# ConsenSys/wittgenstein

Hardware: NVIDIA H100
Metric: simulated-ms/sec, GSFSignature 65,536 nodes (higher is better)
Workload: dtype u64 bitmaps / int32

## Files before the change

wittgenstein_b200/csrc/wtg_cuda.cu:

```cuda
#include <cuda_runtime.h>
#include <unistd.h>

#include <cstdio>
#include <cstdlib>
#include <stdexcept>
#include <string>
#include <vector>

#include "wtg_engine.hpp"

namespace wtg {

#define CUDA_OK(x)                                                                                       \
  do {                                                                                                   \
    cudaError_t e_ = (x);                                                                                \
    if (e_ != cudaSuccess) throw std::runtime_error(std::string("CUDA: ") + cudaGetErrorString(e_) + " at " #x); \
  } while (0)

constexpr int SCAN_THREADS = 256;
constexpr int SCAN_ITEMS = 4;
constexpr int SCAN_TILE = SCAN_THREADS * SCAN_ITEMS;

__global__ void k_begin(Dev d, int mode, bool condAhead) {
  if (threadIdx.x >= 32) return;
  if (d.ffwd && mode == 1) {
    CoopWarp c;
    tickBeginFfwd(d, c);
  } else if (d.farCap > 0 && !d.ffwd) {
    CoopWarp c;
    tickBeginFar(d, c, mode, condAhead);
  } else if (threadIdx.x == 0) {
    tickBegin(d, mode, condAhead);
  }
}
__global__ void k_end(Dev d, int mode, bool condAhead) {
  if (threadIdx.x == 0) tickEnd(d, mode, condAhead);
}
__global__ void k_cond_begin(Dev d) {
  if (threadIdx.x == 0) condBegin(d);
}

__device__ __forceinline__ void listAppend(const Dev& d, bool active, int n, int* cnt, int* list, u64* words = nullptr, u64 word = 0) {
  CoopWarp c;
  unsigned m = c.ballot(active);
  if (!m) return;
  int stripe = ((blockIdx.x * blockDim.x + threadIdx.x) >> 5) & (ARENA_STRIPES - 1);
  int base = 0;
  if (c.lane() == 0) base = atomicAdd(&cnt[stripe], c.count(m));
  base = c.bcast(base, 0);
  if (active) {
    size_t at = (size_t)stripe * d.listStripeCap + base + c.rank(m);
    list[at] = n;
    if (words) words[at] = word;
  }
}
__global__ void __launch_bounds__(256) k_cond_mark(Dev d) {
  if (d.ctl->error) return;
  const int blk = blockIdx.x;
  int n = d.n0 + blk * blockDim.x + threadIdx.x;
  bool due = false;
  if (n < d.n0 + d.nLoc) due = d.proto == PROTO_HANDEL ? hCondMark(d, n) : gsfCondMark(d, n);
  listAppend(d, due, n, d.ctl->dueCnt, d.dueList);
}
template <int PHASE>
__global__ void __launch_bounds__(256) k_cond_nodes(Dev d) {
  extern __shared__ uint32_t keepAll[];
  __shared__ HScratch scratch[8];
  if (d.ctl->error) return;
  const int blk = blockIdx.x, nBlk = gridDim.x;
  const int stripe = blk & (ARENA_STRIPES - 1);
  const int cnt = d.ctl->dueCnt[stripe];
  const int warp = threadIdx.x >> 5;
  const int sub = (blk >> 6) * 8 + warp;
  const int nsub = (nBlk >> 6) * 8;
  const int* list = d.dueList + (size_t)stripe * d.listStripeCap;
  CoopWarp c;
  for (int t = sub; t < cnt; t += nsub) {
    int n = list[t];
    if (PHASE == 0) {
      if (d.proto == PROTO_HANDEL)
        hCondScanQueue(d, c, n);
      else
        gsfCondScanQueue(d, c, n);
    } else {
      if (d.proto == PROTO_HANDEL)
        hCondSelect(d, c, n, &scratch[warp]);
      else
        gsfCondSelect(d, c, n, keepAll + (size_t)warp * (size_t)(d.qcap / 32));
    }
  }
}
__global__ void __launch_bounds__(256) k_cond_score(Dev d) {
  if (d.ctl->error) return;
  const int blk = blockIdx.x, nBlk = gridDim.x;
  const int per = d.workCap / ARENA_STRIPES;
  const int stripe = blk & (ARENA_STRIPES - 1);
  int cnt = d.ctl->workCnt[stripe];
  if (cnt > per) cnt = per;
  const int warpsPerBlock = blockDim.x >> 5;
  const int sub = (blk >> 6) * warpsPerBlock + (threadIdx.x >> 5);
  const int nsub = (nBlk >> 6) * warpsPerBlock;
  CoopWarp c;
  const uint32_t* wl = d.workList + (size_t)stripe * per;
  for (int t = sub; t < cnt; t += nsub) {
    uint32_t it = wl[t];
    if (d.proto == PROTO_HANDEL)
      hScoreItem(d, c, it);
    else
      gsfScoreItem(d, c, it);
  }
}
__global__ void k_hpick_check(Dev d) {
  if (d.ctl->error) return;
  const int blk = blockIdx.x, nBlk = gridDim.x;
  for (int n = d.n0 + blk * blockDim.x + threadIdx.x; n < d.n0 + d.nLoc; n += nBlk * blockDim.x)
    if (d.hCandK[n] > 0 && (d.forcePickSerial || hCondPick(d, n, (u64)d.hDrawBase[n], false) > d.condDraws[n])) d.ctl->hReject = 1;
}
__global__ void k_hpick_apply(Dev d) {
  if (d.ctl->error) return;
  const int blk = blockIdx.x, nBlk = gridDim.x;
  if (!d.ctl->hReject) {
    for (int n = d.n0 + blk * blockDim.x + threadIdx.x; n < d.n0 + d.nLoc; n += nBlk * blockDim.x) hCondPick(d, n, (u64)d.hDrawBase[n], true);
  } else if (blk == 0 && threadIdx.x == 0) {
    u64 idx = 0;
    for (int n = d.n0; n < d.n0 + d.nLoc; ++n) idx += (u64)hCondPick(d, n, idx, true);
  }
}
__global__ void k_hpick_publish(Dev d) {
  const int blk = blockIdx.x, nBlk = gridDim.x;
  if (!d.ctl->error)
    for (int n = d.n0 + blk * blockDim.x + threadIdx.x; n < d.n0 + d.nLoc; n += nBlk * blockDim.x) hPickPublish(d, n);
  if (blk == 0 && threadIdx.x == 0) hPickPublishHeader(d);
}
__global__ void k_hpick_xcheck(Dev d) {
  if (d.ctl->error) return;
  const int blk = blockIdx.x, nBlk = gridDim.x;
  if (blk == 0 && threadIdx.x == 0) hPickHeaders(d);
  const int upTo = hPicksBelow(d, d.rank + 1);
  for (int t = blk * blockDim.x + threadIdx.x; t < upTo; t += nBlk * blockDim.x)
    if (hPickRejects(d, t)) d.ctl->hReject = 1;
}
__global__ void k_hpick_xapply(Dev d) {
  if (d.ctl->error) return;
  const int blk = blockIdx.x, nBlk = gridDim.x;
  if (!d.ctl->hReject) {
    const u64 below = (u64)hPicksBelow(d, d.rank);
    for (int n = d.n0 + blk * blockDim.x + threadIdx.x; n < d.n0 + d.nLoc; n += nBlk * blockDim.x) hCondPick(d, n, below + (u64)d.hDrawBase[n], true);
  } else if (blk == 0 && threadIdx.x == 0) {
    hPickSerial(d);
  }
// ... 383 lines not shown
  }
}
__global__ void __launch_bounds__(256) k_ms_scatter(Dev d) {
  extern __shared__ int msHist[];
  if (d.ctl->error) return;
  const int blk = blockIdx.x, nBlk = gridDim.x;
  const int G = d.ctl->totalSlots, tick = d.ctl->tick, ring = d.ring;
  const int W = d.msWarps, CH = W * MS_SUB;
  const int nChunks = (G + CH - 1) / CH;
  const int warp = threadIdx.x >> 5, lane = threadIdx.x & 31;
  int* base = msHist + warp * ring;
  CoopWarp cw;
  for (int ch = blk; ch < nChunks; ch += nBlk) {
    msZero(msHist, ring, W);
    __syncthreads();
    const int g0 = ch * CH + warp * MS_SUB;
    int tg[MS_ROUNDS];
    msWarpHistogram(d, base, g0, G, tick, lane, tg);
    __syncthreads();
    const int* row = d.msCount + (size_t)ch * ring;
    for (int b = threadIdx.x; b < ring; b += blockDim.x) {
      int run = row[b];
      for (int w = 0; w < W; ++w) {
        int c = msHist[w * ring + b];
        msHist[w * ring + b] = run;
        run += c;
      }
    }
    __syncthreads();
#pragma unroll
    for (int r = 0; r < MS_ROUNDS; ++r) {
      int g = g0 + r * 32 + lane;
      int t = tg[r];
      int pos = cw.claim(base, t - tick, t >= 0);
      if (t >= 0) {
        if (pos < d.bcap) {
          const int4* src = reinterpret_cast<const int4*>(d.newEv + g);
          int4* dst = reinterpret_cast<int4*>(d.buckets + (size_t)(t & (ring - 1)) * (size_t)d.bcap + pos);
          int4 x = src[0], y = src[1];
          dst[0] = x;
          dst[1] = y;
          if (d.G > 1) d.bucketKey[(size_t)(t & (ring - 1)) * (size_t)d.bcap + pos] = orderKey((unsigned)d.ctl->xseq, (unsigned)g);
        }
        if (d.G > 1) d.newTarget[g] = -1;
      }
      __syncwarp();
    }
    __syncthreads();
  }
}

__global__ void k_free(Dev d) {
  if (d.ctl->error) return;
  const int blk = blockIdx.x, nBlk = gridDim.x;
  const int per = d.freeCap / ARENA_STRIPES;
  const int stripe = blk & (ARENA_STRIPES - 1);
  int cnt = d.ctl->freeCnt[stripe];
  if (cnt > per) cnt = per;
  const int sub = (blk >> 6) * blockDim.x + threadIdx.x;
  const int nsub = (nBlk >> 6) * blockDim.x;
  for (int j = sub; j < cnt; j += nsub) freeApply(d, stripe * per + j);
}

__global__ void k_gsf_init_nodes(Dev d) {
  int n = d.n0 + blockIdx.x * blockDim.x + threadIdx.x;
  if (n < d.n0 + d.nLoc) gsfInitNodeBody(d, n);
}
__global__ void k_rng_candidates(Dev d, u64 s0, u64 count, u64 chunk, int maxBound, u64* out, int* outCount, int cap) {
  u64 t = (u64)blockIdx.x * blockDim.x + threadIdx.x;
  u64 start = t * chunk;
  if (start >= count) return;
  u64 len = start + chunk <= count ? chunk : count - start;
  rngCandidateChunk(d, s0, start, len, maxBound, out, outCount, cap);
}
template <class PeerT>
__global__ void k_gsf_shuffle(Dev d, int l, u64 s0, const int* liveRank, const u64* rejOrd, int nRej) {
  int n = d.n0 + blockIdx.x * blockDim.x + threadIdx.x;
  if (n < d.n0 + d.nLoc) gsfShuffleLevel<PeerT>(d, n, l, s0, liveRank, rejOrd, nRej);
}

class CudaBackend : public Backend {
 public:
  cudaStream_t st = nullptr;
  cudaStream_t side = nullptr;
  cudaEvent_t forkEv = nullptr, joinEv = nullptr;
  int devId = 0;
  void bind() const { cudaSetDevice(devId); }
  int sms = 132;
  int smemOptin = 0;
  enum { SHAPE_PLAIN, SHAPE_FIRST, SHAPE_LAST, SHAPE_MIDDLE, NSHAPES };
  cudaGraphExec_t tickGraph[NSHAPES] = {};
  long long shapeKernels[NSHAPES] = {};
  const void* graphFor = nullptr;
  bool useGraph = true;
  long long launches = 0;
  cudaEvent_t tm0 = nullptr, tm1 = nullptr;
  enum ProfSlot { P_BEGIN, P_COND_SCAN, P_DISPATCH_COUNT, P_SCAN_PARTIAL, P_EXCHANGE, P_SCAN_FINAL, P_DISPATCH_SCATTER, P_NODE,
                  P_EMIT, P_MS_COUNT, P_MS_SCAN, P_MS_SCATTER, P_FREE, P_END, P_COND_SCORE, P_COND_SELECT, P_EMIT_PEERS,
                  P_SCAN_A_PARTIAL, P_SCAN_A_FINAL, NK };
  bool profiling = false;
  bool profSplitScans = false;
  std::vector<cudaEvent_t> evPool;
  std::vector<int> evKernel;
  size_t evUsed = 0;
  double profMs[NK] = {};
  long long profCnt[NK] = {};
  const char* profNames[NK] = {"k_begin", "k_cond_scan", "k_dispatch_count", "k_scan_partial", "k_exchange", "k_scan_final",
                               "k_dispatch_scatter", "k_node", "k_emit", "k_ms_count", "k_ms_scan", "k_ms_scatter", "k_free",
                               "k_end", "k_cond_score", "k_cond_select", "k_emit_peers", "k_scan_a_partial", "k_scan_a_final"};

  explicit CudaBackend(int requested = -1) {
    int dev = 0;
    const char* e = std::getenv("LOCAL_RANK");
    int cnt = 0;
    CUDA_OK(cudaGetDeviceCount(&cnt));
    if (cnt == 0) throw std::runtime_error("no CUDA device");
    if (e) dev = std::atoi(e) % cnt;
    const char* e2 = std::getenv("WTG_DEVICE");
    if (e2) dev = std::atoi(e2) % cnt;
    if (requested >= 0) {
      if (requested >= cnt) throw std::invalid_argument("CUDA device " + std::to_string(requested) + " does not exist");
      dev = requested;
    }
    CUDA_OK(cudaSetDevice(dev));
    devId = dev;
    cudaDeviceProp p;
    CUDA_OK(cudaGetDeviceProperties(&p, dev));
    sms = p.multiProcessorCount;
    CUDA_OK(cudaStreamCreateWithFlags(&st, cudaStreamNonBlocking));
    CUDA_OK(cudaStreamCreateWithFlags(&side, cudaStreamNonBlocking));
    CUDA_OK(cudaEventCreateWithFlags(&forkEv, cudaEventDisableTiming));
    CUDA_OK(cudaEventCreateWithFlags(&joinEv, cudaEventDisableTiming));
    CUDA_OK(cudaDeviceGetAttribute(&smemOptin, cudaDevAttrMaxSharedMemoryPerBlockOptin, dev));
    CUDA_OK(cudaFuncSetAttribute(k_ms_count, cudaFuncAttributeMaxDynamicSharedMemorySize, smemOptin));
    CUDA_OK(cudaFuncSetAttribute(k_ms_scatter, cudaFuncAttributeMaxDynamicSharedMemorySize, smemOptin));
    const char* g = std::getenv("WTG_NO_GRAPH");
    if (g && g[0] == '1') useGraph = false;
  }
  ~CudaBackend() override {
    for (void* q : ipcOpened) cudaIpcCloseMemHandle(q);
    for (cudaGraphExec_t g : tickGraph)
      if (g) cudaGraphExecDestroy(g);
    if (forkEv) cudaEventDestroy(forkEv);
    if (joinEv) cudaEventDestroy(joinEv);
    if (side) cudaStreamDestroy(side);
    if (st) cudaStreamDestroy(st);
  }
  void* alloc(size_t bytes) override {
    bind();
    void* p = nullptr;
    cudaError_t e = cudaMalloc(&p, bytes);
    if (e != cudaSuccess) throw std::runtime_error("cudaMalloc of " + std::to_string(bytes) + " bytes failed: " + cudaGetErrorString(e));
    CUDA_OK(cudaMemsetAsync(p, 0, bytes, st));
    return p;
  }
  void release(void* p) override { cudaFree(p); }
  int deviceId() const override { return devId; }
  void exportShared(void* p, unsigned char* handle) override {
    bind();
    std::memset(handle, 0, 128);
    cudaIpcMemHandle_t ih;
    CUDA_OK(cudaIpcGetMemHandle(&ih, p));
// ... 80 lines not shown
    for (int i = 0; i < shown && k < cap; ++i, ++k) {
      ms[k] = profMs[i];
      cnt[k] = profCnt[i];
      names[k] = profNames[i];
      const int a = i == P_SCAN_PARTIAL ? P_SCAN_A_PARTIAL : i == P_SCAN_FINAL ? P_SCAN_A_FINAL : -1;
      if (!profSplitScans && a >= 0) {
        ms[k] += profMs[a];
        cnt[k] += profCnt[a];
      }
    }
    return k;
  }
  void drainProfile() {
    for (size_t i = 0; i < evUsed; ++i) {
      float ms = 0;
      cudaEventElapsedTime(&ms, evPool[2 * i], evPool[2 * i + 1]);
      profMs[evKernel[i]] += ms;
      profCnt[evKernel[i]] += 1;
    }
    evUsed = 0;
  }
  void profBegin(int kid) {
    if (!profiling) return;
    if (evUsed * 2 + 2 > evPool.size()) {
      if (evUsed >= 8192) {
        CUDA_OK(cudaStreamSynchronize(st));
        drainProfile();
      } else {
        cudaEvent_t a, b;
        CUDA_OK(cudaEventCreate(&a));
        CUDA_OK(cudaEventCreate(&b));
        evPool.push_back(a);
        evPool.push_back(b);
        evKernel.push_back(0);
      }
    }
    evKernel[evUsed] = kid;
    CUDA_OK(cudaEventRecord(evPool[2 * evUsed], st));
  }
  void profEnd() {
    if (!profiling) return;
    CUDA_OK(cudaEventRecord(evPool[2 * evUsed + 1], st));
    ++evUsed;
  }

  void fork() {
    CUDA_OK(cudaEventRecord(forkEv, st));
    CUDA_OK(cudaStreamWaitEvent(side, forkEv, 0));
  }
  void join() {
    CUDA_OK(cudaEventRecord(joinEv, side));
    CUDA_OK(cudaStreamWaitEvent(st, joinEv, 0));
  }
  void enqueueCond(const Dev& d, cudaStream_t s) {
    const int wide = sms * 8;
    const size_t smem8 = d.proto == PROTO_GSF ? (size_t)8 * (size_t)(d.qcap / 32) * sizeof(uint32_t) : 0;
    profBegin(P_COND_SCAN);
    k_cond_mark<<<(d.nLoc + 255) / 256, 256, 0, s>>>(d);
    k_cond_nodes<0><<<ARENA_STRIPES * 19, 256, 0, s>>>(d);
    profEnd();
    profBegin(P_COND_SCORE);
    k_cond_score<<<ARENA_STRIPES * 19, 256, 0, s>>>(d);
    profEnd();
    profBegin(P_COND_SELECT);
    k_cond_nodes<1><<<ARENA_STRIPES * 19, 256, smem8, s>>>(d);
    profEnd();
    launches += 4;
    if (d.proto == PROTO_HANDEL) {
      Dev dd = d;
      dd.scanPartial = d.drawScanPartial;
      profBegin(P_SCAN_PARTIAL);
      k_scan_partial<<<wide, SCAN_THREADS, 0, s>>>(dd, 2);
      profEnd();
      profBegin(P_SCAN_FINAL);
      k_scan_final<<<wide, SCAN_THREADS, 0, s>>>(dd, 2);
      profEnd();
      if (d.G > 1) {
        profBegin(P_EXCHANGE);
        k_hpick_publish<<<sms, 256, 0, s>>>(d);
        k_x_sync<<<1, 32, 0, s>>>(d, 3);
        profEnd();
        profBegin(P_COND_SELECT);
        k_hpick_xcheck<<<sms, 256, 0, s>>>(d);
        k_hpick_xapply<<<sms, 256, 0, s>>>(d);
        profEnd();
        launches += 5;
      } else {
        profBegin(P_COND_SELECT);
        k_hpick_check<<<sms, 256, 0, s>>>(d);
        k_hpick_apply<<<sms, 256, 0, s>>>(d);
        profEnd();
        launches += 3;
      }
    }
  }
  void enqueueTick(const Dev& d, int mode, bool ownCond = true, bool nextCond = false) {
    const int wide = sms * 8;
    const size_t msSmem = (size_t)d.msWarps * d.ring * sizeof(int);
    const bool branches = mode == 1 && !profiling && d.G == 1 && (d.proto == PROTO_GSF || d.proto == PROTO_HANDEL);
    const bool condBranch = branches && ownCond;
    cudaStream_t sd = condBranch ? side : st;
    if (mode != 3) {
      profBegin(P_BEGIN);
      k_begin<<<1, 32, 0, st>>>(d, mode, !ownCond);
      profEnd();
    }
    if (condBranch) fork();
    if ((d.proto == PROTO_GSF || d.proto == PROTO_HANDEL) && mode != 3 && ownCond) enqueueCond(d, st);
    if (mode != 2 && mode != 3) {
      profBegin(P_DISPATCH_COUNT);
      k_dispatch_count<<<wide, 256, 0, sd>>>(d);
      profEnd();
      profBegin(P_SCAN_A_PARTIAL);
      k_scan_partial<<<wide, SCAN_THREADS, 0, sd>>>(d, 0);
      profEnd();
      profBegin(P_SCAN_A_FINAL);
      k_scan_final<<<wide, SCAN_THREADS, 0, sd>>>(d, 0);
      profEnd();
      profBegin(P_DISPATCH_SCATTER);
      k_dispatch_scatter<<<wide, 256, 0, sd>>>(d);
      profEnd();
      if (condBranch) join();
      profBegin(P_NODE);
      k_node_msgs<<<(d.nLoc + 255) / 256, 256, 0, st>>>(d);
      k_node_tasks<<<ARENA_STRIPES * 19, 256, 0, st>>>(d);
      if (d.proto == PROTO_CASPER) {
        k_casper_fixups<<<1, 32, 0, st>>>(d);
        launches += 1;
      }
      profEnd();
      launches += 6;
    }
    const bool pooled = d.proto == PROTO_GSF || d.proto == PROTO_HANDEL;
    if (nextCond) {
      fork();
      k_free<<<ARENA_STRIPES * 2, 256, 0, side>>>(d);
      k_cond_begin<<<1, 1, 0, side>>>(d);
      enqueueCond(d, side);
      launches += 2;
    }
    profBegin(P_SCAN_PARTIAL);
    k_scan_partial<<<wide, SCAN_THREADS, 0, st>>>(d, 1);
    profEnd();
    profBegin(P_SCAN_FINAL);
    k_scan_final<<<wide, SCAN_THREADS, 0, st>>>(d, 1);
    profEnd();
    if (d.G > 1) {
      profBegin(P_EXCHANGE);
      k_x1_publish<<<sms * 2, 256, 0, st>>>(d);
      k_x_sync<<<1, 32, 0, st>>>(d, 0);
      k_x1_totals<<<1, 1, 0, st>>>(d);
      k_x1_offsets<<<sms * 2, 256, 0, st>>>(d);
      profEnd();
      launches += 4;
    }
    profBegin(P_EMIT);
    if (d.shufCap > 0) {
      k_shuffle_check<<<ARENA_STRIPES * 4, 256, 0, st>>>(d);
      k_shuffle_serial<<<1, 1, 0, st>>>(d);
      launches += 2;
    }
    k_emit<<<ARENA_STRIPES * 16, 256, 0, st>>>(d);
    if (d.allCap > 0) {
      if (d.G > 1)
        k_x_all_publish<<<8, 128, 0, st>>>(d);
      else
        k_emit_all<<<d.allWarps / 4, 128, 0, st>>>(d);
      launches += 1;
    }
    profEnd();
    if (d.proto == PROTO_P2PFLOOD) {
      profBegin(P_EMIT_PEERS);
      k_emit_peers<<<sms * 8, 128, 0, st>>>(d);
      profEnd();
      launches += 1;
    }
    if (d.G > 1) {
      profBegin(P_EXCHANGE);
      k_x_sync<<<1, 32, 0, st>>>(d, 1);
      k_x2_ingest<<<sms * 4, 256, 0, st>>>(d);
      launches += 2;
      if (d.allCap > 0) {
        k_x_all_build<<<d.allWarps / 4, 128, 0, st>>>(d);
        launches += 1;
      }
      profEnd();
    }
    if (branches && !nextCond) fork();
    profBegin(P_MS_COUNT);
    k_ms_count<<<sms * 2, d.msWarps * 32, msSmem, st>>>(d);
    profEnd();
    profBegin(P_MS_SCAN);
// ... 116 lines not shown
```

wittgenstein_b200/csrc/wtg_engine.hpp:

```cpp
#pragma once
#include <chrono>
#include <cstdio>
#include <functional>
#include <thread>
#include <cstdlib>
#include <cstring>
#include <memory>
#include <string>
#include <vector>

#include "wtg_host.hpp"
#include "wtg_logic.cuh"
#include "wtg_types.h"

namespace wtg {

struct GsfParams {
  int nodeCount, threshold, pairingTime, timeoutPerLevelMs, periodDurationMs, acceleratedCallsCount, nodesDown;
};

struct SfParams {
  int nodeCount, threshold, pairingTime, signatureSize, replyTimeout, candidateCount;
};

// ... 1506 lines not shown
      int fan = 0;
      if (hs.sendTime != 0) {
        if (hs.sendTime <= time) throw std::invalid_argument("sendTime <= time");
        ds.aux |= DESC_SENDTIME;
        ds.target = hs.sendTime;
      }
      if (hs.delay < 0 || hs.delay >= (1 << 20)) throw std::invalid_argument("delaysBetweenMessage");
      if (hs.delay > 0 && hs.to.size() < 2) throw std::invalid_argument("a delay between messages needs several destinations");
      ds.aux |= (uint32_t)hs.delay << DESC_DELAY_SHIFT;
      if (hs.to.empty()) {
        if (d.allCap <= 0) throw std::logic_error("sendAll from the host needs a protocol with the sendAll path (CasperIMD)");
        ds.dkind = DK_SEND_ALL;
        ds.evKind = EV_MULTI;
        ds.nDest = (uint32_t)d.N;
        ds.target = hs.sendTime != 0 ? hs.sendTime : time + 1;
        ds.aux = 0;
        allList.push_back(i);
        fan = d.N;
      } else if (hs.to.size() == 1) {
        if (hs.to[0] < 0 || hs.to[0] >= d.N) throw std::invalid_argument("The to node is not in the network");
        ds.dkind = DK_SEND_SINGLE;
        ds.to = (uint32_t)hs.to[0];
        ds.nDest = 1;
        fan = 1;
      } else {
        ds.dkind = DK_SEND_MULTI;
        ds.to = (uint32_t)scratch.size();
        ds.nDest = (uint32_t)hs.to.size();
        for (int t : hs.to) {
          if (t < 0 || t >= d.N) throw std::invalid_argument("The to node is not in the network");
          scratch.push_back((uint32_t)t);
        }
        if ((int)hs.to.size() > MAX_ACC) scratch.insert(scratch.end(), hs.to.size(), 0u);
        fan = (int)hs.to.size();
      }
      descs[(size_t)i] = ds;
      sent[(size_t)hs.from] += fan;
      bytes[(size_t)hs.from] += (long long)fan * msgSizeOf(hs.meta);
    }
    if ((int)scratch.size() > d.destScratchCap || (int)allList.size() > d.allCap)
      throw std::runtime_error("too many destinations in one call");
    c.tick = time;
    c.condMode = 0;
    c.nEv = 0;
    c.nItems = n;
    c.totalSlots = c.totalDraws = 0;
    c.hReject = 0;
    c.shufReject = 0;
    c.allCnt = (int)allList.size();
    c.nextEvent = 0;
    const int per = d.descCap / ARENA_STRIPES;
    for (int t = 0; t < ARENA_STRIPES; ++t) {
      c.descCnt[t] = std::max(0, std::min(per, n - t * per));
      c.destCnt[t] = c.workCnt[t] = c.dueCnt[t] = c.taskCnt[t] = 0;
    }
    be->upload(d.desc, descs.data(), descs.size() * sizeof(Desc));
    std::vector<int> ones((size_t)n, 1), zerosN((size_t)d.N, 0);
    be->upload(d.evSlots, ones.data(), ones.size() * sizeof(int));
    be->upload(d.evDraws, ones.data(), ones.size() * sizeof(int));
    be->upload(d.condFired + condHalf(d, time), zerosN.data(), zerosN.size() * sizeof(int));
    if (!scratch.empty()) be->upload(d.destScratch, scratch.data(), scratch.size() * sizeof(uint32_t));
    if (!allList.empty()) be->upload(d.allList, allList.data(), allList.size() * sizeof(int));
    {
      std::vector<long long> ms((size_t)d.N), bs((size_t)d.N);
      be->download(ms.data(), d.msgSent, ms.size() * sizeof(long long));
      be->download(bs.data(), d.bytesSent, bs.size() * sizeof(long long));
      for (int i = 0; i < d.N; ++i) {
        ms[(size_t)i] += sent[(size_t)i];
        bs[(size_t)i] += bytes[(size_t)i];
      }
      be->upload(d.msgSent, ms.data(), ms.size() * sizeof(long long));
      be->upload(d.bytesSent, bs.data(), bs.size() * sizeof(long long));
    }
    writeCtl(c);
    be->tick(d, 3);
    c = readCtl();
    if (c.error) throwDeviceError(c);
  }

  int runMs(int ms) {
    requireInited();
    if (sharded() && !linked) throw std::logic_error("node-sharded network: link the shards' exchange regions before runMs");
    if (ms <= 0) throw std::invalid_argument("Should be greater than 0. ms=" + std::to_string(ms));
    long long endAt = (long long)time + ms;
    if (endAt > 0x7fffffffLL) throw std::runtime_error("Maximum time reached!");
    Ctl c = readCtl();
    if (c.error) throwDeviceError(c);
    c.until = (int)endAt;
    c.callId += 1;
    c.didSomething = 0;
    if (d.ffwd) {
      if (c.nextEvent > endAt) {
        c.time = (int)endAt;
        writeCtl(c);
        time = (int)endAt;
        return 0;
      }
      c.idle = 0;
      writeCtl(c);
      int grow = 8;
      for (long long done = 0;;) {
        int batch = (int)std::min<long long>(grow, std::max<long long>(1, ms - done));
        if (grow < 64) grow *= 2;
        runWindow(0, batch, 0);
        done += batch;
        c = readCtl();
        if (c.error) throwDeviceError(c);
        if (c.idle) break;
// ... 234 lines not shown
```

wittgenstein_b200/csrc/wtg_logic.cuh:

```cuda
#pragma once
#include "wtg_types.h"

template <class T, class U>
static inline T wtg_host_fetch_add(T* p, U v) {
  T o = *p;
  *p = (T)(o + (T)v);
  return o;
}
template <class T>
static inline T wtg_host_fetch_max(T* p, T v) {
  T o = *p;
  if (v > o) *p = v;
  return o;
}
template <class T>
static inline T wtg_host_fetch_min(T* p, T v) {
  T o = *p;
  if (v < o) *p = v;
  return o;
}
template <class T>
static inline T wtg_host_cas(T* p, T a, T b) {
  T o = *p;
  if (o == a) *p = b;
// ... 352 lines not shown
}
#if defined(__CUDACC__)
__device__ __forceinline__ void poolCounts(CoopWarp& c, const u64* sig, const u64* rowV, const u64* rowI, int nw, int& cWI, int& cWIV,
                                           int& inter, int& interI) {
  const ulonglong2* s2 = reinterpret_cast<const ulonglong2*>(sig);
  const ulonglong2* v2 = reinterpret_cast<const ulonglong2*>(rowV);
  const ulonglong2* i2 = reinterpret_cast<const ulonglong2*>(rowI);
  const int n2 = nw >> 1;
  for (int w0 = c.lane(); w0 < n2; w0 += 128) {
    ulonglong2 sv[4], vv[4], iv[4];
#pragma unroll
    for (int u = 0; u < 4; ++u) {
      int w = w0 + 32 * u;
      if (w < n2) {
        sv[u] = s2[w];
        vv[u] = v2[w];
        iv[u] = i2[w];
      } else {
        sv[u] = make_ulonglong2(0, 0);
        vv[u] = sv[u];
        iv[u] = sv[u];
      }
    }
#pragma unroll
    for (int u = 0; u < 4; ++u) {
      cWI += __popcll(iv[u].x | sv[u].x) + __popcll(iv[u].y | sv[u].y);
      cWIV += __popcll(iv[u].x | sv[u].x | vv[u].x) + __popcll(iv[u].y | sv[u].y | vv[u].y);
      inter |= ((sv[u].x & vv[u].x) | (sv[u].y & vv[u].y)) != 0;
      interI |= ((sv[u].x & iv[u].x) | (sv[u].y & iv[u].y)) != 0;
    }
  }
}
#endif

template <class C>
WTG_HD int gsfScorePool(const Dev& d, C& c, int n, uint32_t from, uint32_t meta, u64 pl) {
  int l = (int)metaLevel(meta);
  int size = 1 << (l - 1);
  int cV = d.cntVer[n * d.L + l];
  if (cV >= size) return 0;
  Blk b = levelBlock((int)from, l);
  const u64* rowV = d.verified + (size_t)n * d.W64 + b.w0;
  const u64* rowI = d.indivVer + (size_t)n * d.W64 + b.w0;
  const u64* sig = d.pool[l] + (size_t)(uint32_t)pl * (size_t)b.nw;
  int cWI = 0, cWIV = 0, inter = 0, interI = 0;
  poolCounts(c, sig, rowV, rowI, b.nw, cWI, cWIV, inter, interI);
  cWI = c.sum(cWI);
  cWIV = c.sum(cWIV);
  bool bi = c.any(inter != 0), bii = c.any(interI != 0);
  return gsfScoreFrom(l, size, cV, (int)(pl >> 32), bi, cWI, cWIV, bii);
}

WTG_HD size_t condHalf(const Dev& d, int tick) { return (size_t)(tick & 1) * (size_t)d.condStride; }
WTG_HD bool gsfCondMark(const Dev& d, int n) {
  const Ctl& ctl = *d.ctl;
  bool dueNow = false;
  if (ctl.condMode != 0 && !d.ndown[n]) {
    int ms = d.minStart[n];
    bool due = ctl.condMode == 1 ? (ms <= ctl.condTick) : (ms <= ctl.until);
    if (due && d.stamp[n] != ctl.condCall) {
      d.stamp[n] = ctl.condCall;
      if (d.qLen[n] > 0) {
        dueNow = true;
        d.minStart[n] = ctl.condTick + d.pairing[n];
        statAdd(d, n, ST_CONDRUNS, 1ULL);
      }
    }
  }
  d.condDue[n] = dueNow ? 1 : 0;
  if (!dueNow) d.condFired[condHalf(d, ctl.condTick) + n] = 0;
  return dueNow;
}

constexpr int COND_UNROLL = 4;
template <class C>
WTG_HD void gsfCondScanQueue(const Dev& d, C& c, int n) {
  int len = d.qLen[n];
  QEntry* q = d.queue + (size_t)n * d.qcap;
  int* qsc = d.qScore + (size_t)n * d.qcap;
  uint32_t* qst = d.qStamp + (size_t)n * d.qcap;
  const uint32_t* ver = d.lvVer + (size_t)n * d.L;
  const int st = n & (ARENA_STRIPES - 1);
  const int per = d.workCap / ARENA_STRIPES;
  int reeval = 0;
  const int myL = c.lane() < d.L ? c.lane() : 0;
  const int verMine = (int)ver[myL];
  const int cvMine = d.cntVer[n * d.L + myL], ciMine = d.cntIndiv[n * d.L + myL], cuMine = d.cntUnion[n * d.L + myL];
  for (int base0 = 0; base0 < len; base0 += C::LANES * COND_UNROLL) {
    QEntry e[COND_UNROLL];
    uint32_t es[COND_UNROLL];
#pragma unroll
    for (int u = 0; u < COND_UNROLL; ++u) {
      int i = base0 + u * C::LANES + c.lane();
      if (i < len) {
        e[u] = q[i];
        es[u] = qst[i];
      } else {
        e[u].from = 0;
        e[u].meta = 0;
        e[u].pl = 0;
        es[u] = 0;
      }
    }
#pragma unroll
    for (int u = 0; u < COND_UNROLL; ++u) {
      int i = base0 + u * C::LANES + c.lane();
      bool stalePool = false;
      const int lv = (int)metaLevel(e[u].meta);
      const uint32_t v = (uint32_t)c.gather(verMine, lv, reinterpret_cast<const int*>(ver));
      const int cV = c.gather(cvMine, lv, d.cntVer + n * d.L), cI = c.gather(ciMine, lv, d.cntIndiv + n * d.L),
                cU = c.gather(cuMine, lv, d.cntUnion + n * d.L);
      if (i < len) {
        if (es[u] != v) {
          ++reeval;
          if (metaKind(e[u].meta) == PK_POOL) {
            stalePool = true;
          } else {
            qsc[i] = gsfScoreScalarC(d, n, e[u], cV, cI, cU);
            qst[i] = v;
          }
        }
      }
      uint32_t pm = c.ballot(stalePool);
      if (pm) {
        int cnt = c.count(pm), off = c.rank(pm);
        int b0 = 0;
        if (c.lane() == 0) b0 = WTG_ATOMIC_ADD(&d.ctl->workCnt[st], cnt);
        b0 = c.bcast(b0, 0);
        if (stalePool) {
          if (b0 + off < per)
            d.workList[(size_t)st * per + b0 + off] = (uint32_t)((size_t)n * d.qcap + i);
          else
            setError(d, ERR_DESC_OVERFLOW, -n);
        }
      }
    }
  }
  reeval = c.sum(reeval);
  if (c.lane() == 0) {
    statAdd(d, n, ST_EVALENTRIES, (unsigned long long)len);
    statAdd(d, n, ST_EVALPOOL, (unsigned long long)reeval);
  }
}

template <class C>
WTG_HD void gsfScoreItem(const Dev& d, C& c, uint32_t item) {
  int n = (int)(item / (uint32_t)d.qcap);
  QEntry e = d.queue[item];
  int s = gsfScorePool(d, c, n, e.from, e.meta, e.pl);
  if (c.lane() == 0) {
    d.qScore[item] = s;
    d.qStamp[item] = d.lvVer[(size_t)n * d.L + metaLevel(e.meta)];
    statAdd(d, n, ST_EVALWORDS, (unsigned long long)(3 * poolWords((int)metaLevel(e.meta))));
  }
}

template <class C>
WTG_HD void gsfCondSelect(const Dev& d, C& c, int n, uint32_t* keepBits) {
  const Ctl& ctl = *d.ctl;
  int len = d.qLen[n];
  const int pairing = d.pairing[n];
  QEntry* q = d.queue + (size_t)n * d.qcap;
  int* qsc = d.qScore + (size_t)n * d.qcap;
  uint32_t* qst = d.qStamp + (size_t)n * d.qcap;
  int bestScore = 0, bestIdx = 0x7fffffff;
  for (int base0 = 0; base0 < len; base0 += C::LANES * COND_UNROLL) {
    int sc[COND_UNROLL];
#pragma unroll
    for (int u = 0; u < COND_UNROLL; ++u) {
      int i = base0 + u * C::LANES + c.lane();
      sc[u] = i < len ? qsc[i] : 0;
    }
#pragma unroll
    for (int u = 0; u < COND_UNROLL; ++u) {
      int base = base0 + u * C::LANES;
      if (base >= len) break;
      int i = base + c.lane();
      uint32_t km = c.ballot(sc[u] > 0);
      if (c.lane() == 0) keepBits[base / C::LANES] = km;
      if (sc[u] > bestScore) {
        bestScore = sc[u];
        bestIdx = i;
      }
    }
  }
  int mx = c.maxv(bestScore);
  int bi = c.minv(bestScore == mx ? bestIdx : 0x7fffffff);
  bool found = mx > 0;
  c.sync();
  QEntry best;
  best.from = 0;
  best.meta = 0;
  best.pl = 0;
  int w = 0;
  int base0 = 0;
// ... 1295 lines not shown
        farAppend(d, ev, target, g);
      target = -1;
    }
  } else if (target >= 0 && target - ctl.tick >= d.ring) {
    setError(d, ERR_FAR_FUTURE, target);
    target = -1;
  }
  if (shard) {
    if (target >= 0) xStoreEnvelope(d, ownerOf(d, (int)ev.to), g, ev, target);
    return;
  }
  d.newEv[g] = ev;
  d.newTarget[g] = target;
}

WTG_HD void emitCond(const Dev& d, int n) {
  const size_t h = condHalf(d, d.ctl->tick);
  if (!d.condFired[h + n]) return;
  int g = d.slotBase[n - d.n0];
  if (d.G > 1) g += d.ctl->condXoffS;
  if (g >= d.newEvCap) {
    setError(d, ERR_DESC_OVERFLOW, g);
    return;
  }
  int target = d.condTarget[h + n];
  if (target - d.ctl->tick >= d.ring) {
    setError(d, ERR_FAR_FUTURE, target);
    target = -1;
  }
  if (d.G > 1 && target < 0) return;
  d.newEv[g] = d.condEv[h + n];
  d.newTarget[g] = target;
}

WTG_HD void tickBegin(const Dev& d, int mode, bool condAhead = false) {
  Ctl& c = *d.ctl;
  if (mode == 1) {
    c.time += 1;
    c.tick = c.time;
    c.condMode = 1;
    c.nEv = d.bucketCount[c.tick & (d.ring - 1)];
  } else if (mode == 0) {
    c.tick = c.time;
    c.condMode = 0;
    c.nEv = d.bucketCount[c.tick & (d.ring - 1)];
  } else {
    c.tick = c.time + 1;
    c.condMode = 2;
    c.nEv = 0;
  }
  for (int t = 0; t < ARENA_STRIPES; ++t) {
    c.descCnt[t] = 0;
    c.destCnt[t] = 0;
    if (!condAhead) {
      c.workCnt[t] = 0;
      c.dueCnt[t] = 0;
    }
    c.taskCnt[t] = 0;
  }
  if (!condAhead) {
    c.condTick = c.tick;
    c.condCall = c.callId;
  }
  c.nItems = 0;
  c.totalSlots = 0;
  c.totalDraws = 0;
  c.hReject = 0;
  c.allCnt = 0;
  c.shufReject = 0;
  c.peerCnt = 0;
  if (c.nEv > c.maxBucket) c.maxBucket = c.nEv;
  if (d.G > 1) {
    c.xseq += 1;
    c.nEvGlobal = 0;
    for (int q = 0; q < MAX_SHARDS; ++q) c.stageTop[q] = 0;
  }
}
template <class C>
WTG_HD void tickBeginFar(const Dev& d, C& c, int mode, bool condAhead = false) {
  if (mode != 2) farMigrate(d, c, mode == 1 ? d.ctl->time + 1 : d.ctl->time);
  c.sync();
  if (c.lane() == 0) tickBegin(d, mode, condAhead);
  c.sync();
}
WTG_HD void samplePoolMinFree(const Dev& d) {
  Ctl& c = *d.ctl;
  if (d.proto == PROTO_GSF && (c.tick & 15) == 0)
    for (int l = INLINE_MAX_LEVEL + 1; l < d.L; ++l) {
      int f = 0;
      for (int t = 0; t < POOL_STRIPES; ++t) f += c.poolFreeCnt[l][t];
      if (f < c.poolMinFree[l]) c.poolMinFree[l] = f;
    }
}
WTG_HD void tickEnd(const Dev& d, int mode, bool condAhead = false) {
  Ctl& c = *d.ctl;
  c.rng = lcgAdvance(d.jumpA, d.jumpC, c.rng, (u64)c.totalDraws);
  c.statDraws += (unsigned long long)c.totalDraws;
  c.statEvents += (unsigned long long)c.nItems;
  if ((d.G > 1 ? c.nEvGlobal : c.nEv) > 0) {
    c.callId += 1;
    c.didSomething = 1;
  }
  if (mode != 2 && mode != 3) d.bucketCount[c.tick & (d.ring - 1)] = 0;
  for (int t = 0; t < ARENA_STRIPES; ++t) c.freeCnt[t] = 0;
  if (d.proto == PROTO_CASPER && d.G > 1 && d.cg->createdThisTick > 1) setError(d, ERR_UNSUPPORTED, 4);
  if (d.G > 1 && d.allCap > 0 && mode != 3) c.allSeq = (int)(((unsigned)c.allSeq + (unsigned)xAllTotal(d)) & 0x3fffffffu);
  if (!condAhead) samplePoolMinFree(d);
}
WTG_HD void condBegin(const Dev& d) {
  Ctl& c = *d.ctl;
  samplePoolMinFree(d);
  c.condTick = c.tick + 1;
  c.condCall = c.callId + (c.nEv > 0 ? 1u : 0u);
  c.condMode = 1;
  for (int t = 0; t < ARENA_STRIPES; ++t) {
    c.workCnt[t] = 0;
    c.dueCnt[t] = 0;
  }
}
WTG_HD void freeApply(const Dev& d, int i) {
  uint32_t w = d.freeList[i];
  freeDirect(d, (int)(w >> 27), w & 0x7FFFFFFu);
}
WTG_HD int stripedIndex(const int* cnt, int per, int t) {
  for (int s = 0; s < ARENA_STRIPES; ++s) {
    int c = cnt[s];
    if (c > per) c = per;
    if (t < c) return s * per + t;
    t -= c;
  }
  return -1;
}
WTG_HD int stripedTotal(const int* cnt, int per) {
  int tot = 0;
  for (int s = 0; s < ARENA_STRIPES; ++s) tot += cnt[s] > per ? per : cnt[s];
  return tot;
}

WTG_HD void gsfInitNodeBody(const Dev& d, int n) {
  d.verified[(size_t)n * d.W64 + (n >> 6)] = 1ULL << (n & 63);
  d.totalCard[n] = 1;
  d.minStart[n] = 1;
  if (!d.ndown[n]) {
    d.cntVer[n * d.L] = 1;
    d.cntUnion[n * d.L] = 1;
    for (int l = 1; l < d.L; ++l) d.remaining[n * d.L + l] = 1 << (l - 1);
  }
  for (int l = 0; l < d.L; ++l) d.lvVer[n * d.L + l] = 1;
}

WTG_HD void rngCandidateChunk(const Dev& d, u64 s0, u64 start, u64 len, int maxBound, u64* out, int* outCount, int cap) {
  u64 s = lcgAdvance(d.jumpA, d.jumpC, s0, start);
  const uint32_t thr = 0x80000000u - (uint32_t)maxBound;
  for (u64 i = 0; i < len; ++i) {
    s = (s * 0x5DEECE66DULL + 0xBULL) & LCG_MASK;
    uint32_t u = (uint32_t)(s >> 17);
    if (u >= thr) {
      int k = WTG_ATOMIC_ADD(outCount, 1);
      if (k < cap) out[k] = start + i;
    }
  }
}

template <class PeerT>
WTG_HD void gsfShuffleLevel(const Dev& d, int n, int l, u64 s0, const int* liveRank, const u64* rejOrd, int nRej) {
  int r = liveRank[n];
  if (r < 0) return;
// ... 101 lines not shown
```

wittgenstein_b200/csrc/wtg_types.h:

```cpp
#pragma once
#include <stdint.h>

#if defined(__CUDACC__)
#define WTG_HD __host__ __device__ __forceinline__
#else
#define WTG_HD inline
#endif

namespace wtg {

constexpr int POOL_STRIPES = 64;
constexpr int ARENA_STRIPES = 64;
constexpr int MS_SUB_ENVELOPES = 256;
constexpr int MAX_LEVELS = 24;
constexpr int MAX_ACC = 16;
constexpr int INLINE_MAX_LEVEL = 7;
constexpr int MAX_DIST = 1144;
constexpr int MAX_SHARDS = 8;

enum : int { PROTO_NONE = 0, PROTO_PINGPONG = 1, PROTO_GSF = 2, PROTO_SANFERMIN = 3, PROTO_HANDEL = 4, PROTO_CASPER = 5, PROTO_CAPPOS = 6,
             PROTO_SLUSH = 7, PROTO_SNOWFLAKE = 8, PROTO_P2PFLOOD = 9 };

enum : uint32_t {
  EV_MSG = 0,
// ... 127 lines not shown
constexpr uint32_t META_STAGED = 1u << 15;
constexpr int META_SRC_SHIFT = 16;
struct MultiRec;
struct Ev;
struct Peer {
  XHdr* hdr;
  XItem* items;
  int* flags;
  Ev* newEv;
  int* newTarget;
  unsigned long long* stage;
  MultiRec* rec;
  uint32_t* recDest;
  int* recArrival;
  XBegin* beg;
  XAll* all;
  int* allCnt;
  char* proto;
};

struct CasperG {
  int nBlocks;
  int byzToSend, byzH, byzLate, byzOnTime;
  int createdThisTick;
  int byzDirect, byzOlder, byzNotBest, byzSkipped;
  int pad[2];
};

struct Ctl {
  int time;
  int until;
  int tick;
  int condMode;
  int nEv;
  int nItems;
  int totalSlots, totalDraws;
  uint32_t callId;
  int didSomething;
  unsigned long long rng;
  int error;
  int errorDetail;
  int recTop, recDestTop;
  int hReject;
  int farCnt, farMin;
  int idle;
  int nextEvent;
  int allCnt;
  int shufReject;
  int maxBucket;
  unsigned long long statDraws, statEvents;
  int descCnt[ARENA_STRIPES];
  int destCnt[ARENA_STRIPES];
  int freeCnt[ARENA_STRIPES];
  int workCnt[ARENA_STRIPES];
  int dueCnt[ARENA_STRIPES];
  int taskCnt[ARENA_STRIPES];
  int xseq;
  int nEvGlobal;
  int condXoffS, condXoffD;
  int allCondS, allCondD;
  int stageTop[MAX_SHARDS];
  int xRecTop[MAX_SHARDS];
  int xRecDestTop[MAX_SHARDS];
  int tieCnt;
  int allSeq;
  int xNext, xAfter;
  int poolMinFree[MAX_LEVELS];
  int poolFreeCnt[MAX_LEVELS][POOL_STRIPES];
  long long serialPasses;
  int peerCnt;
  int condTick;
  uint32_t condCall;
};

enum : int {
  ST_DELIVERIES = 0, ST_TASKS, ST_CONDRUNS, ST_EVALENTRIES, ST_EVALWORDS, ST_UPDATES, ST_CYCLES, ST_SENDS, ST_MULTISENDS,
  ST_SENDWORDS, ST_EVALPOOL, ST_UPDATEWORDS, ST_MAXQUEUE, ST_MAXINBOX, ST_COUNT = 16
};
constexpr int STAT_SLOTS = 1024;

enum : int {
  ERR_NONE = 0,
  ERR_BUCKET_OVERFLOW = 1,
  ERR_QUEUE_OVERFLOW = 2,
  ERR_POOL_EXHAUSTED = 3,
  ERR_FAR_FUTURE = 4,
  ERR_DESC_OVERFLOW = 5,
  ERR_REC_OVERFLOW = 6,
  ERR_FREE_OVERFLOW = 7,
  ERR_INTERNAL = 8,
  ERR_INBOX_OVERFLOW = 9,
  ERR_FAR_OVERFLOW = 10,
  ERR_PROTO_STATE = 11,
  ERR_UNSUPPORTED = 12,
  ERR_PEER_TIMEOUT = 13,
  ERR_PEER_ERROR = 14,
  ERR_STAGE_OVERFLOW = 15
};

struct Dev {
  int N, L, W64;
  int ring;
  int msChunks;
  int msWarps;
  int proto;
  int threshold, timeoutPerLevel, period, accel;
  int qcap, bcap;
  int msgDiscardTime;
  int descCap, destScratchCap, recCap, recDestCap, freeCap, newEvCap, itemCap, workCap;
  int latKind, latParam;
  int peerBits;
  int n0, nLoc, G, rank, ownShift;
  int xItemCap, stageCapWords, xRecCap, xRecDestCap;
  int perShard;
  int xAllCap;
  Peer peer[MAX_SHARDS];
  unsigned long long* bucketKey;
  unsigned long long* itemKey;
  uint32_t* xoffS;
  uint32_t* xoffD;
  Ctl* ctl;
  unsigned long long* stats;
  int16_t* nx;
  int16_t* ny;
  int16_t* nextra;
// ... 173 lines not shown
```

Before: 5176.

## Fuse free and cond-begin into ahead cond-mark kernel with double-buffered counters

On the side stream, the separate k_free and single-thread k_cond_begin launches are folded into a templated k_cond_mark<true>. It frees stripes first, uses a grid-wide atomic counter so the last block samples pool min-free, and computes the cond clock locally. The work and due counters are doubled so the ahead set lives in its own half, and the begin/end ticks reset both halves. This removes two launches and a serial single-thread kernel from the overlapped branch, at the cost of an atomic last-block handshake and a more complex ordering contract between free and mark.

```diff
diff --git a/wittgenstein_b200/csrc/wtg_cuda.cu b/wittgenstein_b200/csrc/wtg_cuda.cu
--- a/wittgenstein_b200/csrc/wtg_cuda.cu
+++ b/wittgenstein_b200/csrc/wtg_cuda.cu
@@ -36,8 +36,24 @@
 __global__ void k_end(Dev d, int mode, bool condAhead) {
   if (threadIdx.x == 0) tickEnd(d, mode, condAhead);
 }
-__global__ void k_cond_begin(Dev d) {
-  if (threadIdx.x == 0) condBegin(d);
+__device__ __forceinline__ void freeStripes(const Dev& d) {
+  const int blk = blockIdx.x, nBlk = gridDim.x;
+  const int per = d.freeCap / ARENA_STRIPES;
+  if (nBlk >= ARENA_STRIPES) {
+    if (blk >= nBlk / ARENA_STRIPES * ARENA_STRIPES) return;
+    const int stripe = blk & (ARENA_STRIPES - 1);
+    int cnt = d.ctl->freeCnt[stripe];
+    if (cnt > per) cnt = per;
+    const int sub = (blk >> 6) * blockDim.x + threadIdx.x;
+    const int nsub = (nBlk >> 6) * blockDim.x;
+    for (int j = sub; j < cnt; j += nsub) freeApply(d, stripe * per + j);
+  } else {
+    for (int stripe = blk; stripe < ARENA_STRIPES; stripe += nBlk) {
+      int cnt = d.ctl->freeCnt[stripe];
+      if (cnt > per) cnt = per;
+      for (int j = threadIdx.x; j < cnt; j += blockDim.x) freeApply(d, stripe * per + j);
+    }
+  }
 }
 
 __device__ __forceinline__ void listAppend(const Dev& d, bool active, int n, int* cnt, int* list, u64* words = nullptr, u64 word = 0) {
@@ -54,22 +70,37 @@
     if (words) words[at] = word;
   }
 }
+template <bool AHEAD>
 __global__ void __launch_bounds__(256) k_cond_mark(Dev d) {
-  if (d.ctl->error) return;
-  const int blk = blockIdx.x;
-  int n = d.n0 + blk * blockDim.x + threadIdx.x;
+  CondClock clk;
+  if (AHEAD) {
+    if (!d.ctl->error) freeStripes(d);
+    __threadfence();
+    __syncthreads();
+    if (threadIdx.x == 0 && atomicAdd(&d.ctl->markDone, 1) == (int)gridDim.x - 1) {
+      __threadfence();
+      samplePoolMinFree(d);
+      d.ctl->markDone = 0;
+    }
+    clk = condClockAhead(*d.ctl);
+    if (blockIdx.x == 0 && threadIdx.x == 0) condClockStore(d, clk);
+  } else {
+    clk = condClockOwn(*d.ctl);
+  }
+  if (d.ctl->error) return;
+  int n = d.n0 + blockIdx.x * blockDim.x + threadIdx.x;
   bool due = false;
-  if (n < d.n0 + d.nLoc) due = d.proto == PROTO_HANDEL ? hCondMark(d, n) : gsfCondMark(d, n);
-  listAppend(d, due, n, d.ctl->dueCnt, d.dueList);
+  if (n < d.n0 + d.nLoc) due = d.proto == PROTO_HANDEL ? hCondMark(d, n) : gsfCondMark(d, n, clk);
+  listAppend(d, due, n, d.ctl->dueCnt + condSet(AHEAD), d.dueList);
 }
 template <int PHASE>
-__global__ void __launch_bounds__(256) k_cond_nodes(Dev d) {
+__global__ void __launch_bounds__(256) k_cond_nodes(Dev d, bool ahead) {
   extern __shared__ uint32_t keepAll[];
   __shared__ HScratch scratch[8];
   if (d.ctl->error) return;
   const int blk = blockIdx.x, nBlk = gridDim.x;
   const int stripe = blk & (ARENA_STRIPES - 1);
-  const int cnt = d.ctl->dueCnt[stripe];
+  const int cnt = d.ctl->dueCnt[condSet(ahead) + stripe];
   const int warp = threadIdx.x >> 5;
   const int sub = (blk >> 6) * 8 + warp;
   const int nsub = (nBlk >> 6) * 8;
@@ -81,7 +112,7 @@
       if (d.proto == PROTO_HANDEL)
         hCondScanQueue(d, c, n);
       else
-        gsfCondScanQueue(d, c, n);
+        gsfCondScanQueue(d, c, n, ahead);
     } else {
       if (d.proto == PROTO_HANDEL)
         hCondSelect(d, c, n, &scratch[warp]);
@@ -90,12 +121,12 @@
     }
   }
 }
-__global__ void __launch_bounds__(256) k_cond_score(Dev d) {
+__global__ void __launch_bounds__(256) k_cond_score(Dev d, bool ahead) {
   if (d.ctl->error) return;
   const int blk = blockIdx.x, nBlk = gridDim.x;
   const int per = d.workCap / ARENA_STRIPES;
   const int stripe = blk & (ARENA_STRIPES - 1);
-  int cnt = d.ctl->workCnt[stripe];
+  int cnt = d.ctl->workCnt[condSet(ahead) + stripe];
   if (cnt > per) cnt = per;
   const int warpsPerBlock = blockDim.x >> 5;
   const int sub = (blk >> 6) * warpsPerBlock + (threadIdx.x >> 5);
@@ -585,14 +616,7 @@
 
 __global__ void k_free(Dev d) {
   if (d.ctl->error) return;
-  const int blk = blockIdx.x, nBlk = gridDim.x;
-  const int per = d.freeCap / ARENA_STRIPES;
-  const int stripe = blk & (ARENA_STRIPES - 1);
-  int cnt = d.ctl->freeCnt[stripe];
-  if (cnt > per) cnt = per;
-  const int sub = (blk >> 6) * blockDim.x + threadIdx.x;
-  const int nsub = (nBlk >> 6) * blockDim.x;
-  for (int j = sub; j < cnt; j += nsub) freeApply(d, stripe * per + j);
+  freeStripes(d);
 }
 
 __global__ void k_gsf_init_nodes(Dev d) {
@@ -630,7 +654,7 @@
   cudaEvent_t tm0 = nullptr, tm1 = nullptr;
   enum ProfSlot { P_BEGIN, P_COND_SCAN, P_DISPATCH_COUNT, P_SCAN_PARTIAL, P_EXCHANGE, P_SCAN_FINAL, P_DISPATCH_SCATTER, P_NODE,
                   P_EMIT, P_MS_COUNT, P_MS_SCAN, P_MS_SCATTER, P_FREE, P_END, P_COND_SCORE, P_COND_SELECT, P_EMIT_PEERS,
-                  P_SCAN_A_PARTIAL, P_SCAN_A_FINAL, NK };
+                  P_COND_MARK, P_SCAN_A_PARTIAL, P_SCAN_A_FINAL, NK };
   bool profiling = false;
   bool profSplitScans = false;
   std::vector<cudaEvent_t> evPool;
@@ -640,7 +664,8 @@
   long long profCnt[NK] = {};
   const char* profNames[NK] = {"k_begin", "k_cond_scan", "k_dispatch_count", "k_scan_partial", "k_exchange", "k_scan_final",
                                "k_dispatch_scatter", "k_node", "k_emit", "k_ms_count", "k_ms_scan", "k_ms_scatter", "k_free",
-                               "k_end", "k_cond_score", "k_cond_select", "k_emit_peers", "k_scan_a_partial", "k_scan_a_final"};
+                               "k_end", "k_cond_score", "k_cond_select", "k_emit_peers", "k_cond_mark", "k_scan_a_partial",
+                               "k_scan_a_final"};
 
   explicit CudaBackend(int requested = -1) {
     int dev = 0;
@@ -827,18 +852,23 @@
     CUDA_OK(cudaEventRecord(joinEv, side));
     CUDA_OK(cudaStreamWaitEvent(st, joinEv, 0));
   }
-  void enqueueCond(const Dev& d, cudaStream_t s) {
+  void enqueueCond(const Dev& d, cudaStream_t s, bool ahead = false) {
     const int wide = sms * 8;
     const size_t smem8 = d.proto == PROTO_GSF ? (size_t)8 * (size_t)(d.qcap / 32) * sizeof(uint32_t) : 0;
+    profBegin(P_COND_MARK);
+    if (ahead)
+      k_cond_mark<true><<<(d.nLoc + 255) / 256, 256, 0, s>>>(d);
+    else
+      k_cond_mark<false><<<(d.nLoc + 255) / 256, 256, 0, s>>>(d);
+    profEnd();
     profBegin(P_COND_SCAN);
-    k_cond_mark<<<(d.nLoc + 255) / 256, 256, 0, s>>>(d);
-    k_cond_nodes<0><<<ARENA_STRIPES * 19, 256, 0, s>>>(d);
+    k_cond_nodes<0><<<ARENA_STRIPES * 19, 256, 0, s>>>(d, ahead);
     profEnd();
     profBegin(P_COND_SCORE);
-    k_cond_score<<<ARENA_STRIPES * 19, 256, 0, s>>>(d);
+    k_cond_score<<<ARENA_STRIPES * 19, 256, 0, s>>>(d, ahead);
     profEnd();
     profBegin(P_COND_SELECT);
-    k_cond_nodes<1><<<ARENA_STRIPES * 19, 256, smem8, s>>>(d);
+    k_cond_nodes<1><<<ARENA_STRIPES * 19, 256, smem8, s>>>(d, ahead);
     profEnd();
     launches += 4;
     if (d.proto == PROTO_HANDEL) {
@@ -909,10 +939,7 @@
     const bool pooled = d.proto == PROTO_GSF || d.proto == PROTO_HANDEL;
     if (nextCond) {
       fork();
-      k_free<<<ARENA_STRIPES * 2, 256, 0, side>>>(d);
-      k_cond_begin<<<1, 1, 0, side>>>(d);
-      enqueueCond(d, side);
-      launches += 2;
+      enqueueCond(d, side, true);
     }
     profBegin(P_SCAN_PARTIAL);
     k_scan_partial<<<wide, SCAN_THREADS, 0, st>>>(d, 1);
diff --git a/wittgenstein_b200/csrc/wtg_engine.hpp b/wittgenstein_b200/csrc/wtg_engine.hpp
--- a/wittgenstein_b200/csrc/wtg_engine.hpp
+++ b/wittgenstein_b200/csrc/wtg_engine.hpp
@@ -1582,8 +1582,9 @@
     const int per = d.descCap / ARENA_STRIPES;
     for (int t = 0; t < ARENA_STRIPES; ++t) {
       c.descCnt[t] = std::max(0, std::min(per, n - t * per));
-      c.destCnt[t] = c.workCnt[t] = c.dueCnt[t] = c.taskCnt[t] = 0;
-    }
+      c.destCnt[t] = c.taskCnt[t] = 0;
+    }
+    for (int t = 0; t < 2 * ARENA_STRIPES; ++t) c.workCnt[t] = c.dueCnt[t] = 0;
     be->upload(d.desc, descs.data(), descs.size() * sizeof(Desc));
     std::vector<int> ones((size_t)n, 1), zerosN((size_t)d.N, 0);
     be->upload(d.evSlots, ones.data(), ones.size() * sizeof(int));
diff --git a/wittgenstein_b200/csrc/wtg_logic.cuh b/wittgenstein_b200/csrc/wtg_logic.cuh
--- a/wittgenstein_b200/csrc/wtg_logic.cuh
+++ b/wittgenstein_b200/csrc/wtg_logic.cuh
@@ -428,29 +428,41 @@
 }
 
 WTG_HD size_t condHalf(const Dev& d, int tick) { return (size_t)(tick & 1) * (size_t)d.condStride; }
-WTG_HD bool gsfCondMark(const Dev& d, int n) {
-  const Ctl& ctl = *d.ctl;
+WTG_HD int condSet(bool ahead) { return ahead ? ARENA_STRIPES : 0; }
+struct CondClock {
+  int mode, tick;
+  uint32_t call;
+};
+WTG_HD CondClock condClockOwn(const Ctl& c) { return CondClock{c.condMode, c.condTick, c.condCall}; }
+WTG_HD CondClock condClockAhead(const Ctl& c) { return CondClock{1, c.tick + 1, c.callId + (c.nEv > 0 ? 1u : 0u)}; }
+WTG_HD void condClockStore(const Dev& d, const CondClock& k) {
+  d.ctl->condMode = k.mode;
+  d.ctl->condTick = k.tick;
+  d.ctl->condCall = k.call;
+}
+WTG_HD bool gsfCondMark(const Dev& d, int n, const CondClock& k) {
   bool dueNow = false;
-  if (ctl.condMode != 0 && !d.ndown[n]) {
+  if (k.mode != 0 && !d.ndown[n]) {
     int ms = d.minStart[n];
-    bool due = ctl.condMode == 1 ? (ms <= ctl.condTick) : (ms <= ctl.until);
-    if (due && d.stamp[n] != ctl.condCall) {
-      d.stamp[n] = ctl.condCall;
+    bool due = k.mode == 1 ? (ms <= k.tick) : (ms <= d.ctl->until);
+    if (due && d.stamp[n] != k.call) {
+      d.stamp[n] = k.call;
       if (d.qLen[n] > 0) {
         dueNow = true;
-        d.minStart[n] = ctl.condTick + d.pairing[n];
+        d.minStart[n] = k.tick + d.pairing[n];
         statAdd(d, n, ST_CONDRUNS, 1ULL);
       }
     }
   }
   d.condDue[n] = dueNow ? 1 : 0;
-  if (!dueNow) d.condFired[condHalf(d, ctl.condTick) + n] = 0;
+  if (!dueNow) d.condFired[condHalf(d, k.tick) + n] = 0;
   return dueNow;
 }
+WTG_HD bool gsfCondMark(const Dev& d, int n) { return gsfCondMark(d, n, condClockOwn(*d.ctl)); }
 
 constexpr int COND_UNROLL = 4;
 template <class C>
-WTG_HD void gsfCondScanQueue(const Dev& d, C& c, int n) {
+WTG_HD void gsfCondScanQueue(const Dev& d, C& c, int n, bool ahead) {
   int len = d.qLen[n];
   QEntry* q = d.queue + (size_t)n * d.qcap;
   int* qsc = d.qScore + (size_t)n * d.qcap;
@@ -458,6 +470,7 @@
   const uint32_t* ver = d.lvVer + (size_t)n * d.L;
   const int st = n & (ARENA_STRIPES - 1);
   const int per = d.workCap / ARENA_STRIPES;
+  int* workCnt = d.ctl->workCnt + condSet(ahead);
   int reeval = 0;
   const int myL = c.lane() < d.L ? c.lane() : 0;
   const int verMine = (int)ver[myL];
@@ -501,7 +514,7 @@
       if (pm) {
         int cnt = c.count(pm), off = c.rank(pm);
         int b0 = 0;
-        if (c.lane() == 0) b0 = WTG_ATOMIC_ADD(&d.ctl->workCnt[st], cnt);
+        if (c.lane() == 0) b0 = WTG_ATOMIC_ADD(&workCnt[st], cnt);
         b0 = c.bcast(b0, 0);
         if (stalePool) {
           if (b0 + off < per)
@@ -517,6 +530,11 @@
     statAdd(d, n, ST_EVALENTRIES, (unsigned long long)len);
     statAdd(d, n, ST_EVALPOOL, (unsigned long long)reeval);
   }
+}
+
+template <class C>
+WTG_HD void gsfCondScanQueue(const Dev& d, C& c, int n) {
+  gsfCondScanQueue(d, c, n, false);
 }
 
 template <class C>
@@ -1918,11 +1936,11 @@
   for (int t = 0; t < ARENA_STRIPES; ++t) {
     c.descCnt[t] = 0;
     c.destCnt[t] = 0;
-    if (!condAhead) {
-      c.workCnt[t] = 0;
-      c.dueCnt[t] = 0;
-    }
     c.taskCnt[t] = 0;
+  }
+  for (int t = 0; t < 2 * ARENA_STRIPES; ++t) {
+    c.workCnt[t] = 0;
+    c.dueCnt[t] = 0;
   }
   if (!condAhead) {
     c.condTick = c.tick;
@@ -1954,7 +1972,7 @@
   if (d.proto == PROTO_GSF && (c.tick & 15) == 0)
     for (int l = INLINE_MAX_LEVEL + 1; l < d.L; ++l) {
       int f = 0;
-      for (int t = 0; t < POOL_STRIPES; ++t) f += c.poolFreeCnt[l][t];
+      for (int t = 0; t < POOL_STRIPES; ++t) f += ((volatile int*)c.poolFreeCnt[l])[t];
       if (f < c.poolMinFree[l]) c.poolMinFree[l] = f;
     }
 }
@@ -1976,9 +1994,7 @@
 WTG_HD void condBegin(const Dev& d) {
   Ctl& c = *d.ctl;
   samplePoolMinFree(d);
-  c.condTick = c.tick + 1;
-  c.condCall = c.callId + (c.nEv > 0 ? 1u : 0u);
-  c.condMode = 1;
+  condClockStore(d, condClockAhead(c));
   for (int t = 0; t < ARENA_STRIPES; ++t) {
     c.workCnt[t] = 0;
     c.dueCnt[t] = 0;
diff --git a/wittgenstein_b200/csrc/wtg_types.h b/wittgenstein_b200/csrc/wtg_types.h
--- a/wittgenstein_b200/csrc/wtg_types.h
+++ b/wittgenstein_b200/csrc/wtg_types.h
@@ -203,8 +203,8 @@
   int descCnt[ARENA_STRIPES];
   int destCnt[ARENA_STRIPES];
   int freeCnt[ARENA_STRIPES];
-  int workCnt[ARENA_STRIPES];
-  int dueCnt[ARENA_STRIPES];
+  int workCnt[2 * ARENA_STRIPES];
+  int dueCnt[2 * ARENA_STRIPES];
   int taskCnt[ARENA_STRIPES];
   int xseq;
   int nEvGlobal;
@@ -222,6 +222,7 @@
   int peerCnt;
   int condTick;
   uint32_t condCall;
+  int markDone;
 };
 
 enum : int {
```

Result: no change. 5168, median of 6 (-0.1%).
